# linyicheng1/keypoint_bench

Hardware: AMD Instinct MI355X
Metric: image-pairs/sec (extract+NMS+BF-match, 640x480, top_k=1000) (higher is better)
Workload: dtype f32

## Files before the change

### keypoint_bench_amd/csrc/match.hip

```cpp
#include "kpb_common.h"

namespace {

struct SampleArgs {
    const float* desc; const float* pts; const int* n; float* out;
    int C, Hd, Wd, pts_cols, max_n;
    long long sb, sc, sh, sw;
};

constexpr int SAMPLE_KPW = 4;
__global__ __launch_bounds__(256) void sample_bilinear(SampleArgs a)
{
    const int b = blockIdx.y, lane = threadIdx.x & 63;
    const int i0 = (blockIdx.x * 4 + (threadIdx.x >> 6)) * SAMPLE_KPW;
    const int n = a.n ? min(a.n[b], a.max_n) : a.max_n;
    if (i0 >= n) return;
    float cf[SAMPLE_KPW][4];
    long long off[SAMPLE_KPW][4];
    bool ok[SAMPLE_KPW][4];
#pragma unroll
    for (int k = 0; k < SAMPLE_KPW; ++k) {
        const int i = min(i0 + k, n - 1);
        const float* p = a.pts + ((size_t)b * a.max_n + i) * a.pts_cols;
        const float gx = (p[0] - 0.5f) * 2.0f, gy = (p[1] - 0.5f) * 2.0f;
        const float x = (gx + 1.0f) * ((float)(a.Wd - 1) / 2.0f), y = (gy + 1.0f) * ((float)(a.Hd - 1) / 2.0f);
        const float xw = floorf(x), yn = floorf(y);
        const float w = x - xw, e = 1.0f - w, nn = y - yn, s = 1.0f - nn;
        cf[k][0] = s * e; cf[k][1] = s * w; cf[k][2] = nn * e; cf[k][3] = nn * w;
        const long long x0 = (long long)xw, y0 = (long long)yn, x1 = x0 + 1, y1 = y0 + 1;
        const bool vx0 = x0 >= 0 && x0 < a.Wd, vx1 = x1 >= 0 && x1 < a.Wd;
        const bool vy0 = y0 >= 0 && y0 < a.Hd, vy1 = y1 >= 0 && y1 < a.Hd;
        ok[k][0] = vx0 && vy0; ok[k][1] = vx1 && vy0; ok[k][2] = vx0 && vy1; ok[k][3] = vx1 && vy1;
        off[k][0] = ok[k][0] ? y0 * a.sh + x0 * a.sw : 0; off[k][1] = ok[k][1] ? y0 * a.sh + x1 * a.sw : 0;
        off[k][2] = ok[k][2] ? y1 * a.sh + x0 * a.sw : 0; off[k][3] = ok[k][3] ? y1 * a.sh + x1 * a.sw : 0;
    }
    const float* base = a.desc + (size_t)b * a.sb;
    for (int ch = lane; ch < a.C; ch += 64) {
        const float* q = base + (size_t)ch * a.sc;
        float t[SAMPLE_KPW][4];
#pragma unroll
        for (int k = 0; k < SAMPLE_KPW; ++k)
#pragma unroll
            for (int c = 0; c < 4; ++c) t[k][c] = q[off[k][c]];
#pragma unroll
        for (int k = 0; k < SAMPLE_KPW; ++k) {
            const float nw = ok[k][0] ? t[k][0] : 0.0f, ne = ok[k][1] ? t[k][1] : 0.0f;
            const float sw = ok[k][2] ? t[k][2] : 0.0f, se = ok[k][3] ? t[k][3] : 0.0f;
            if (i0 + k < n)
                a.out[((size_t)b * a.max_n + i0 + k) * a.C + ch] =
                    __fadd_rn(__fadd_rn(__fadd_rn(__fmul_rn(nw, cf[k][0]), __fmul_rn(ne, cf[k][1])), __fmul_rn(sw, cf[k][2])), __fmul_rn(se, cf[k][3]));
        }
    }
}

__device__ __forceinline__ bool precedes(double s1, int i1, double s2, int i2)
{
    if (s1 == s2) return i1 < i2;
    const bool n1 = s1 != s1, n2 = s2 != s2;
    if (n1 | n2) return n1 && (!n2 || i1 < i2);
    const double hi = fmax(s1, s2), lo = fmin(s1, s2);
    if (hi - lo <= hi * 4.5e-16) {
        const double d1 = sqrt(s1), d2 = sqrt(s2);
        if (d1 == d2) return i1 < i2;
        return d1 < d2;
    }
    return s1 < s2;
}

constexpr int TM = 4, TN = 8;
constexpr int MTI = 16 * TM, MTJ = 16 * TN, KC = 16, MATCH_THREADS = 256;

struct MatchArgs {
    const int* only;
    const float* d0; const float* d1; const int* n; const int* m;
    double* rpart_s; int* rpart_j;
    double* cpart_s; int* cpart_i;
    int C, max_n, max_m, tiles_i, rdepth;
};

__host__ __device__ constexpr int row_depth(int tiles_j) { return 2 * tiles_j > 8 ? 2 * tiles_j : 8; }

#define COLJ(c, q) (2 * (c) + 32 * ((q) >> 1) + ((q) & 1))
template <bool RATIO>
__global__ __launch_bounds__(MATCH_THREADS) void match_tile(MatchArgs a)
{
    constexpr int PA = MTI + 2, PB = MTJ + 2;
    constexpr int STAGE = KC * (PA + PB) * 2, RED = 16 * MTJ * 3;
    __shared__ __attribute__((aligned(16))) unsigned smem[STAGE > RED ? STAGE : RED];
    double (*A)[PA] = reinterpret_cast<double (*)[PA]>(smem);
    double (*Bt)[PB] = reinterpret_cast<double (*)[PB]>(smem + KC * PA * 2);
    const int b = blockIdx.z, tj = blockIdx.x, ti = blockIdx.y, tid = threadIdx.x;
    if (a.only && !a.only[b]) return;
    const int n = a.n ? min(a.n[b], a.max_n) : a.max_n, m = a.m ? min(a.m[b], a.max_m) : a.max_m;
    const int i0 = ti * MTI, j0 = tj * MTJ;
    if (i0 >= n || j0 >= m) return;
    const float* d0 = a.d0 + (size_t)b * a.max_n * a.C;
    const float* d1 = a.d1 + (size_t)b * a.max_m * a.C;
    const int r = tid >> 4, c = tid & 15;
    double acc[TM][TN];
#pragma unroll
    for (int p = 0; p < TM; ++p)
#pragma unroll
        for (int q = 0; q < TN; ++q) acc[p][q] = 0.0;

    const bool vec = (a.C % 4) == 0;
    for (int k0 = 0; k0 < a.C; k0 += KC) {
        if (vec) {
            for (int x = tid; x < (MTI + MTJ) * (KC / 4); x += MATCH_THREADS) {
                const int row = x / (KC / 4), kq = x - row * (KC / 4), kk = k0 + 4 * kq;
                const bool second = row >= MTI;
                const int lr = second ? row - MTI : row;
                const float* src = second ? d1 + (size_t)min(j0 + lr, m - 1) * a.C : d0 + (size_t)min(i0 + lr, n - 1) * a.C;
                float4 v = make_float4(0.f, 0.f, 0.f, 0.f);
                if (kk < a.C) v = *reinterpret_cast<const float4*>(src + kk);
                double* dst = second ? &Bt[4 * kq][lr] : &A[4 * kq][lr];
                const int pitch = second ? PB : PA;
                dst[0] = (double)v.x; dst[pitch] = (double)v.y; dst[2 * pitch] = (double)v.z; dst[3 * pitch] = (double)v.w;
            }
        } else {
            for (int x = tid; x < (MTI + MTJ) * KC; x += MATCH_THREADS) {
                const int row = x % (MTI + MTJ), k = x / (MTI + MTJ), kk = k0 + k;
                if (row < MTI) A[k][row] = (kk < a.C) ? (double)d0[(size_t)min(i0 + row, n - 1) * a.C + kk] : 0.0;
                else Bt[k][row - MTI] = (kk < a.C) ? (double)d1[(size_t)min(j0 + row - MTI, m - 1) * a.C + kk] : 0.0;
            }
        }
        __syncthreads();
        const int kend = min(KC, a.C - k0);
        for (int k = 0; k < kend; ++k) {
            double av[TM], bv[TN];
#pragma unroll
            for (int p = 0; p < TM; ++p) av[p] = A[k][TM * r + p];
#pragma unroll
            for (int q = 0; q < TN; ++q) bv[q] = Bt[k][COLJ(c, q)];
#pragma unroll
            for (int p = 0; p < TM; ++p)
#pragma unroll
                for (int q = 0; q < TN; ++q) {
                    const double d = __dsub_rn(av[p], bv[q]);
                    acc[p][q] = __dadd_rn(acc[p][q], __dmul_rn(d, d));
                }
        }
        __syncthreads();
    }

    const int lane = tid & 63;
#pragma unroll
    for (int p = 0; p < TM; ++p) {
        double bs = __longlong_as_double(0x7FF0000000000000LL);
        int bj = 0x7FFFFFFF;
        double ss = bs;
        int sj = bj;
#pragma unroll
        for (int q = 0; q < TN; ++q) {
            const int j = j0 + COLJ(c, q);
            if (j < m) {
                if (precedes(acc[p][q], j, bs, bj)) {
                    if (RATIO) { ss = bs; sj = bj; }
                    bs = acc[p][q]; bj = j;
                } else if (RATIO && precedes(acc[p][q], j, ss, sj)) { ss = acc[p][q]; sj = j; }
            }
        }
#pragma unroll
        for (int d = 1; d < 16; d <<= 1) {
            const double os = __shfl_xor(bs, d, 64);
            const int oj = __shfl_xor(bj, d, 64);
            if (RATIO) {
                const double os2 = __shfl_xor(ss, d, 64);
                const int oj2 = __shfl_xor(sj, d, 64);
                if (precedes(os, oj, bs, bj)) {
                    if (precedes(os2, oj2, bs, bj)) { ss = os2; sj = oj2; } else { ss = bs; sj = bj; }
                    bs = os; bj = oj;
                } else if (precedes(os, oj, ss, sj)) { ss = os; sj = oj; }
            } else if (precedes(os, oj, bs, bj)) { bs = os; bj = oj; }
        }
        const int i = i0 + TM * r + p;
        if ((lane & 15) == 0 && i < n) {
            const size_t o = ((size_t)b * a.rdepth + (RATIO ? 2 * tj : tj)) * a.max_n + i;
            a.rpart_s[o] = bs; a.rpart_j[o] = bj;
            if (RATIO) { a.rpart_s[o + a.max_n] = ss; a.rpart_j[o + a.max_n] = sj; }
        }
    }
    double (*cs)[MTJ] = reinterpret_cast<double (*)[MTJ]>(smem);
    int (*ci)[MTJ] = reinterpret_cast<int (*)[MTJ]>(smem + 16 * MTJ * 2);
#pragma unroll
    for (int q = 0; q < TN; ++q) {
        double bs = __longlong_as_double(0x7FF0000000000000LL);
        int bi = 0x7FFFFFFF;
#pragma unroll
        for (int p = 0; p < TM; ++p) {
            const int i = i0 + TM * r + p;
            if (i < n && precedes(acc[p][q], i, bs, bi)) { bs = acc[p][q]; bi = i; }
        }
        cs[r][COLJ(c, q)] = bs; ci[r][COLJ(c, q)] = bi;
    }
    __syncthreads();
    if (tid < MTJ) {
        double bs = cs[0][tid]; int bi = ci[0][tid];
        for (int g = 1; g < 16; ++g)
            if (precedes(cs[g][tid], ci[g][tid], bs, bi)) { bs = cs[g][tid]; bi = ci[g][tid]; }
        const int j = j0 + tid;
        if (j < m) {
            const size_t o = ((size_t)b * a.tiles_i + ti) * a.max_m + j;
            a.cpart_s[o] = bs; a.cpart_i[o] = bi;
        }
    }
}

constexpr int FIN_THREADS = 1024;

struct FinArgs {
    const double* rpart_s; const int* rpart_j; const double* cpart_s; const int* cpart_i;
    const int* n; const int* m;
    int* out_pairs; double* out_dist; int* out_k;
    int* host_k;
    int max_n, max_m, tiles_i, rdepth, cross_check;
    double max_distance;
    const int* exact;
    double max_ratio;
};

template <bool RATIO>
__global__ __launch_bounds__(FIN_THREADS) void match_finalize(FinArgs a)
{
    extern __shared__ __attribute__((aligned(16))) unsigned char smem[];
    int* colarg = reinterpret_cast<int*>(smem);
    __shared__ int wsum[FIN_THREADS / 64];
    const int b = blockIdx.x, tid = threadIdx.x, lane = tid & 63, wid = tid >> 6;
    const int n = a.n ? min(a.n[b], a.max_n) : a.max_n, m = a.m ? min(a.m[b], a.max_m) : a.max_m;
    const int tiles_i = (n + MTI - 1) / MTI;
    const int rslots = !RATIO ? (m + MTJ - 1) / MTJ : (a.exact && !a.exact[b]) ? a.rdepth : 2 * ((m + MTJ - 1) / MTJ);
    for (int j = tid; j < m; j += FIN_THREADS) {
        double bs = __longlong_as_double(0x7FF0000000000000LL);
        int bi = 0x7FFFFFFF;
        for (int t = 0; t < tiles_i; ++t) {
            const size_t o = ((size_t)b * a.tiles_i + t) * a.max_m + j;
            const double s = a.cpart_s[o]; const int i = a.cpart_i[o];
            if (i != 0x7FFFFFFF && precedes(s, i, bs, bi)) { bs = s; bi = i; }
        }
        colarg[j] = bi;
    }
    __syncthreads();
    int base = 0;
    for (int c0 = 0; c0 < n; c0 += FIN_THREADS) {
        const int i = c0 + tid;
        bool keep = false;
        double dist = 0.0;
        int bj = 0;
        if (i < n && m > 0) {
            double bs = __longlong_as_double(0x7FF0000000000000LL);
            bj = 0x7FFFFFFF;
            int bt = 0;
            for (int t = 0; t < rslots; ++t) {
                const size_t o = ((size_t)b * a.rdepth + t) * a.max_n + i;
                const double s = a.rpart_s[o]; const int j = a.rpart_j[o];
                if (j != 0x7FFFFFFF && precedes(s, j, bs, bj)) { bs = s; bj = j; bt = t; }
            }
            dist = sqrt(bs);
            keep = (!a.cross_check || colarg[bj] == i) && (!(a.max_distance < __longlong_as_double(0x7FF0000000000000LL)) || dist < a.max_distance);
            if (RATIO && keep) {
                double ss = __longlong_as_double(0x7FF0000000000000LL);
                int sj = 0x7FFFFFFF;
                for (int t = 0; t < rslots; ++t) {
                    const size_t o = ((size_t)b * a.rdepth + t) * a.max_n + i;
                    const double s = a.rpart_s[o]; const int j = a.rpart_j[o];
                    if (t != bt && j != 0x7FFFFFFF && precedes(s, j, ss, sj)) { ss = s; sj = j; }
                }
                double second = sqrt(ss);
                if (second == 0.0) second = 2.220446049250313e-16;
                keep = __ddiv_rn(dist, second) < a.max_ratio;
            }
        }
        const unsigned long long bal = __ballot(keep);
        const int within = __popcll(bal & ((1ull << lane) - 1ull));
        if (lane == 0) wsum[wid] = __popcll(bal);
        __syncthreads();
        int wbase = 0, tot = 0;
        for (int w = 0; w < FIN_THREADS / 64; ++w) { const int s = wsum[w]; if (w < wid) wbase += s; tot += s; }
        __syncthreads();
        if (keep) {
            const int pos = base + wbase + within;
            a.out_pairs[((size_t)b * a.max_n + pos) * 2 + 0] = i;
            a.out_pairs[((size_t)b * a.max_n + pos) * 2 + 1] = bj;
            if (a.out_dist) a.out_dist[(size_t)b * a.max_n + pos] = dist;
        }
        base += tot;
    }
    if (tid == 0) { a.out_k[b] = base; a.host_k[b] = base; }
}

typedef _Float16 mh8 __attribute__((ext_vector_type(8)));
typedef float mf4 __attribute__((ext_vector_type(4)));
constexpr unsigned INF_BITS = 0x7F800000u;
__device__ __forceinline__ float match_margin(float na, float nb, int C)
{
    return (7.5e-6f + 6.0e-7f * (float)C) * (na + nb) + 5.0e-6f * (sqrtf(na) + sqrtf(nb));
}

struct PreArgs {
    const float* d0; const float* d1; const int* n; const int* m;
    int C, max_n, max_m;
    uint4* h0; uint4* h1;
    float* nrm0; float* nrm1;
    unsigned* rowmin; unsigned* colmin;
    int* rcnt; int* ccnt;
    int* flag;
    int* ncand;
    unsigned* nmax;
};

__global__ __launch_bounds__(256) void match_prep(PreArgs a)
{
    __shared__ unsigned s_max[2];
    const int b = blockIdx.y, tid = threadIdx.x, q = tid & 7;
    const int n = a.n ? min(a.n[b], a.max_n) : a.max_n, m = a.m ? min(a.m[b], a.max_m) : a.max_m;
    const int P8 = a.C / 8;
    if (tid < 2) s_max[tid] = 0u;
    __syncthreads();
    const int r = min(blockIdx.x * 32 + (tid >> 3), a.max_n + a.max_m - 1);
    const bool second = r >= a.max_n;
    const int row = second ? r - a.max_n : r;
    const int cnt = second ? m : n, cap = second ? a.max_m : a.max_n;
    const float* src = (second ? a.d1 : a.d0) + ((size_t)b * cap + row) * a.C;
    uint4* dst = (second ? a.h1 : a.h0) + ((size_t)b * cap + row) * P8;
    const size_t lo_off = (size_t)gridDim.y * cap * P8;
    float nn = 0.0f, big = 0.0f;
    if (row < cnt) {
        for (int p8 = q; p8 < P8; p8 += 8) {
            const float4 u = *reinterpret_cast<const float4*>(src + 8 * p8), v = *reinterpret_cast<const float4*>(src + 8 * p8 + 4);
            const float f[8] = {u.x, u.y, u.z, u.w, v.x, v.y, v.z, v.w};
            big = fmaxf(fmaxf(fmaxf(big, fmaxf(fabsf(u.x), fabsf(u.y))), fmaxf(fabsf(u.z), fabsf(u.w))),
                        fmaxf(fmaxf(fabsf(v.x), fabsf(v.y)), fmaxf(fabsf(v.z), fabsf(v.w))));
            unsigned hw[4], lw[4];
#pragma unroll
            for (int k = 0; k < 4; ++k) {
                typedef _Float16 h2 __attribute__((ext_vector_type(2)));
                const h2 hh = __builtin_bit_cast(h2, __builtin_amdgcn_cvt_pkrtz(f[2 * k], f[2 * k + 1]));
                const h2 ll = __builtin_bit_cast(h2, __builtin_amdgcn_cvt_pkrtz(f[2 * k] - (float)hh[0], f[2 * k + 1] - (float)hh[1]));
                hw[k] = __builtin_bit_cast(unsigned, hh); lw[k] = __builtin_bit_cast(unsigned, ll);
                nn = fmaf(f[2 * k], f[2 * k], nn); nn = fmaf(f[2 * k + 1], f[2 * k + 1], nn);
            }
            dst[p8] = make_uint4(hw[0], hw[1], hw[2], hw[3]);
            dst[lo_off + p8] = make_uint4(lw[0], lw[1], lw[2], lw[3]);
        }
    }
    nn += kpb_shfl_xor<1>(nn); nn += kpb_shfl_xor<2>(nn); nn += kpb_shfl_xor<4>(nn);
    if (row < cnt && big >= 32768.0f) a.flag[b] = 1;
    if (row < cnt && q == 0) {
        if (!(nn < 3.0e38f)) a.flag[b] = 1;
        else atomicMax(&s_max[second ? 1 : 0], __float_as_uint(nn));
    }
    if (q == 0) {
        (second ? a.nrm1 : a.nrm0)[(size_t)b * cap + row] = nn;
        (second ? a.colmin : a.rowmin)[(size_t)b * cap + row] = INF_BITS;
        (second ? a.ccnt : a.rcnt)[(size_t)b * cap + row] = 0;
    }
    __syncthreads();
    if (tid < 2 && s_max[tid]) atomicMax(&a.nmax[2 * b + tid], s_max[tid]);
}

struct ApxArgs {
    const uint4* h0; const uint4* h1; const float* nrm0; const float* nrm1; const int* n; const int* m;
    int max_n, max_m, P8; size_t lo0, lo1;
    unsigned* rowmin; unsigned* colmin;
    int2* cand; int* ncand; int cap; int* flag;
    const unsigned* nmax; int C;
};

constexpr int CBUF = 192;

template <int KB, int RT, int PASS, bool RATIO = false>
__global__ __launch_bounds__(256) void match_approx(ApxArgs a)
{
    static_assert(PASS == 0 || !RATIO, "the candidate pass is the same with the ratio test on");
    __shared__ int2 cbuf[PASS == 1 ? 4 : 1][PASS == 1 ? CBUF : 1];
    int wcnt = 0;
    const int b = blockIdx.y, tid = threadIdx.x, lane = tid & 63, wv = tid >> 6;
    auto flush = [&]() {
        if (PASS == 1 && wcnt > 0) {
            int base = 0;
            if (lane == 0) base = atomicAdd(&a.ncand[b], wcnt);
            base = __shfl(base, 0, 64);
            for (int i = lane; i < wcnt; i += 64) {
                if (base + i < a.cap) a.cand[(size_t)b * a.cap + base + i] = cbuf[PASS == 1 ? wv : 0][i];
                else a.flag[b] = 1;
            }
            wcnt = 0;
        }
    };
    const int n = a.n ? min(a.n[b], a.max_n) : a.max_n, m = a.m ? min(a.m[b], a.max_m) : a.max_m;
    if (a.flag[b]) return;
    const int i0 = (blockIdx.x * 4 + wv) * (16 * RT);
    if (i0 >= n) return;
    const int c16 = lane & 15, g = lane >> 4;
    const uint4* A = a.h0 + (size_t)b * a.max_n * a.P8;
    const uint4* Bm = a.h1 + (size_t)b * a.max_m * a.P8;
    mh8 ah[RT][KB], al[RT][KB];
    float na[RT][4];
#pragma unroll
    for (int rt = 0; rt < RT; ++rt) {
        const int row = min(i0 + 16 * rt + c16, n - 1);
#pragma unroll
        for (int kb = 0; kb < KB; ++kb) {
            ah[rt][kb] = __builtin_bit_cast(mh8, A[(size_t)row * a.P8 + 4 * kb + g]);
            al[rt][kb] = __builtin_bit_cast(mh8, A[a.lo0 + (size_t)row * a.P8 + 4 * kb + g]);
        }
#pragma unroll
        for (int r = 0; r < 4; ++r) {
            const int i = i0 + 16 * rt + 4 * g + r;
            na[rt][r] = i < n ? a.nrm0[(size_t)b * a.max_n + i] : __uint_as_float(INF_BITS);
        }
    }
    const float namax = __uint_as_float(a.nmax[2 * b]), nbmax = __uint_as_float(a.nmax[2 * b + 1]);
    float rmin[RT][4];
    float rmin2[RATIO ? RT : 1][4];
    if (RATIO) {
#pragma unroll
        for (int rt = 0; rt < RT; ++rt)
#pragma unroll
            for (int r = 0; r < 4; ++r) rmin2[RATIO ? rt : 0][r] = __uint_as_float(INF_BITS);
    }
#pragma unroll
    for (int rt = 0; rt < RT; ++rt)
#pragma unroll
        for (int r = 0; r < 4; ++r) rmin[rt][r] = PASS == 0 ? __uint_as_float(INF_BITS)
                                                             : (i0 + 16 * rt + 4 * g + r < n ? __uint_as_float(a.rowmin[(size_t)b * a.max_n + i0 + 16 * rt + 4 * g + r]) + match_margin(na[rt][r], nbmax, a.C) : -1.0f);
    for (int j0 = 0; j0 < m; j0 += 16) {
        const int j = j0 + c16;
        const int jr = min(j, m - 1);
        mh8 bh[KB], bl[KB];
#pragma unroll
        for (int kb = 0; kb < KB; ++kb) {
            bh[kb] = __builtin_bit_cast(mh8, Bm[(size_t)jr * a.P8 + 4 * kb + g]);
            bl[kb] = __builtin_bit_cast(mh8, Bm[a.lo1 + (size_t)jr * a.P8 + 4 * kb + g]);
        }
        const float nb = j < m ? a.nrm1[(size_t)b * a.max_m + j] : __uint_as_float(INF_BITS);
        const float cmin_j = PASS == 1 && j < m ? __uint_as_float(a.colmin[(size_t)b * a.max_m + j]) + match_margin(namax, nb, a.C) : -1.0f;
        float cm = __uint_as_float(INF_BITS);
#pragma unroll
        for (int rt = 0; rt < RT; ++rt) {
            mf4 acc = {0.f, 0.f, 0.f, 0.f};
#pragma unroll
            for (int kb = 0; kb < KB; ++kb) {
                acc = __builtin_amdgcn_mfma_f32_16x16x32_f16(al[rt][kb], bh[kb], acc, 0, 0, 0);
                acc = __builtin_amdgcn_mfma_f32_16x16x32_f16(ah[rt][kb], bl[kb], acc, 0, 0, 0);
                acc = __builtin_amdgcn_mfma_f32_16x16x32_f16(ah[rt][kb], bh[kb], acc, 0, 0, 0);
            }
            float dd[4];
#pragma unroll
            for (int r = 0; r < 4; ++r)
                dd[r] = fmaxf(__fadd_rn(__fadd_rn(na[rt][r], nb), -2.0f * acc[r]), 0.0f) + 0.0f;
            if (PASS == 0) {
#pragma unroll
                for (int r = 0; r < 4; ++r) {
                    if (RATIO) rmin2[RATIO ? rt : 0][r] = fminf(rmin2[RATIO ? rt : 0][r], fmaxf(rmin[rt][r], dd[r]));
                    rmin[rt][r] = fminf(rmin[rt][r], dd[r]); cm = fminf(cm, dd[r]);
                }
            } else {
                unsigned rowc = 0, colc = 0;
#pragma unroll
                for (int r = 0; r < 4; ++r) {
                    const bool fin = dd[r] < __uint_as_float(INF_BITS);
                    rowc |= (fin && dd[r] <= rmin[rt][r]) ? 1u << r : 0u;
                    colc |= (fin && dd[r] <= cmin_j) ? 1u << r : 0u;
                }
                const unsigned any = rowc | colc;
                if (__ballot(any != 0)) {
#pragma unroll
                    for (int r = 0; r < 4; ++r) {
                        const bool hit = (any >> r) & 1u;
                        const unsigned long long bal = __ballot(hit);
                        if (bal) {
                            if (hit) cbuf[PASS == 1 ? wv : 0][wcnt + __popcll(bal & ((1ull << lane) - 1ull))] =
                                make_int2((i0 + 16 * rt + 4 * g + r) | (((rowc >> r) & 1u) ? 1 << 30 : 0) | (((colc >> r) & 1u) ? 1 << 29 : 0), j);
                            wcnt += __popcll(bal);
                            if (wcnt > CBUF - 64) flush();
                        }
                    }
                }
            }
        }
        if (PASS == 0) {
            cm = fminf(cm, kpb_shfl_xor<16>(cm));
            cm = kpb_min32(cm);
            if (g == 0 && j < m) atomicMin(&a.colmin[(size_t)b * a.max_m + j], __float_as_uint(cm));
        }
    }
    flush();
    if (PASS == 0) {
#pragma unroll
        for (int rt = 0; rt < RT; ++rt)
#pragma unroll
            for (int r = 0; r < 4; ++r) {
                float v = rmin[rt][r];
                if (RATIO) {
                    float w = rmin2[RATIO ? rt : 0][r], ov, ow;
                    ov = kpb_shfl_xor<1>(v); ow = kpb_shfl_xor<1>(w); w = fminf(fmaxf(v, ov), fminf(w, ow)); v = fminf(v, ov);
                    ov = kpb_shfl_xor<2>(v); ow = kpb_shfl_xor<2>(w); w = fminf(fmaxf(v, ov), fminf(w, ow)); v = fminf(v, ov);
                    ov = kpb_shfl_xor<4>(v); ow = kpb_shfl_xor<4>(w); w = fminf(fmaxf(v, ov), fminf(w, ow)); v = fminf(v, ov);
                    ov = kpb_shfl_xor<8>(v); ow = kpb_shfl_xor<8>(w); w = fminf(fmaxf(v, ov), fminf(w, ow));
                    v = w;
                } else {
                    v = fminf(v, kpb_shfl_xor<1>(v)); v = fminf(v, kpb_shfl_xor<2>(v));
                    v = fminf(v, kpb_shfl_xor<4>(v)); v = fminf(v, kpb_shfl_xor<8>(v));
                }
                const int i = i0 + 16 * rt + 4 * g + r;
                if (c16 == 0 && i < n) a.rowmin[(size_t)b * a.max_n + i] = __float_as_uint(v);
            }
    }
}

struct ExactArgs {
    const float* d0; const float* d1; const int2* cand; const int* ncand; int cap, C, max_n, max_m;
    int* rcnt; int* ccnt; double* rs; int* rj; double* cs; int* ci; int tiles_i, rdepth; const int* m; const int* n; int* flag;
    int ratio;
};

__global__ __launch_bounds__(256) void match_exact(ExactArgs a)
{
    const int b = blockIdx.y;
    const int e = blockIdx.x * 256 + threadIdx.x;
    if (a.flag[b] || e >= min(a.ncand[b], a.cap)) return;
    const int2 c = a.cand[(size_t)b * a.cap + e];
    const int i = c.x & 0x1FFFFFFF, j = c.y;
    const float* pa = a.d0 + ((size_t)b * a.max_n + i) * a.C;
    const float* pb = a.d1 + ((size_t)b * a.max_m + j) * a.C;
    double s = 0.0;
    for (int k = 0; k < a.C; k += 4) {
        const float4 u = *reinterpret_cast<const float4*>(pa + k), v = *reinterpret_cast<const float4*>(pb + k);
        double d = __dsub_rn((double)u.x, (double)v.x); s = __dadd_rn(s, __dmul_rn(d, d));
        d = __dsub_rn((double)u.y, (double)v.y); s = __dadd_rn(s, __dmul_rn(d, d));
        d = __dsub_rn((double)u.z, (double)v.z); s = __dadd_rn(s, __dmul_rn(d, d));
        d = __dsub_rn((double)u.w, (double)v.w); s = __dadd_rn(s, __dmul_rn(d, d));
    }
    const int n = a.n ? min(a.n[b], a.max_n) : a.max_n, m = a.m ? min(a.m[b], a.max_m) : a.max_m;
    const int slots_r = a.ratio ? a.rdepth : (m + MTJ - 1) / MTJ, slots_c = (n + MTI - 1) / MTI;
    if (c.x & (1 << 30)) {
        const int t = atomicAdd(&a.rcnt[(size_t)b * a.max_n + i], 1);
        if (t < slots_r) { const size_t o = ((size_t)b * a.rdepth + t) * a.max_n + i; a.rs[o] = s; a.rj[o] = j; }
        else a.flag[b] = 1;
    }
    if (c.x & (1 << 29)) {
        const int t = atomicAdd(&a.ccnt[(size_t)b * a.max_m + j], 1);
        if (t < slots_c) { const size_t o = ((size_t)b * a.tiles_i + t) * a.max_m + j; a.cs[o] = s; a.ci[o] = i; }
        else a.flag[b] = 1;
    }
}

__global__ void gather_rows(const float* src, int src_rows, int cols, const int* idx, int idx_rows, int idx_stride,
                            int idx_col, const int* k, float* out)
{
    const int b = blockIdx.y;
    const int kk = k ? min(k[b], idx_rows) : idx_rows;
    const int e = blockIdx.x * blockDim.x + threadIdx.x;
    const int i = e / cols, c = e - i * cols;
    if (i >= kk) return;
    const int r = idx[((size_t)b * idx_rows + i) * idx_stride + idx_col];
    out[((size_t)b * idx_rows + i) * cols + c] = src[((size_t)b * src_rows + r) * cols + c];
}

}

extern "C" __attribute__((visibility("default"))) int kpb_sample(kpb_ctx* ctx, const float* desc_dev, int batch, int C, int Hd, int Wd, int64_t sb,
                          int64_t sc, int64_t sh, int64_t sw, const float* pts_dev, int pts_cols, int max_n,
                          const int32_t* n_dev, float* out_dev)
{
    if (!ctx) return kpb_fail(nullptr, KPB_E_INVALID, "kpb_sample: null context");
    if (max_n == 0) return KPB_OK;
    if (!desc_dev || !pts_dev || !out_dev || batch <= 0 || C <= 0 || Hd <= 0 || Wd <= 0 || pts_cols < 2 || max_n < 0)
        return kpb_fail(ctx, KPB_E_INVALID, "kpb_sample: bad argument");
    KPB_HIP(ctx, hipSetDevice(ctx->device));
    SampleArgs a{desc_dev, pts_dev, n_dev, out_dev, C, Hd, Wd, pts_cols, max_n, sb, sc, sh, sw};
    KPB_LAUNCH(ctx, "sample_bilinear", sample_bilinear, dim3(cdiv(max_n, 4 * SAMPLE_KPW), batch), dim3(256), 0, ctx->stream, a);
    KPB_HIP(ctx, hipGetLastError());
    return KPB_OK;
}

static int match_impl(kpb_ctx* ctx, const float* d0_dev, const float* d1_dev, int batch, int C, int max_n, int max_m, const int32_t* n_dev,
                      const int32_t* m_dev, const kpb_match_params* prm, double max_ratio, int32_t* out_pairs_dev, double* out_dist_dev, int32_t* out_k_dev)
{
    const bool ratio = max_ratio < 1.0;
    ctx->match_counts_valid = 0;
    if (!prm || !out_k_dev || batch <= 0 || C <= 0 || max_n < 0 || max_m < 0)
        return kpb_fail(ctx, KPB_E_INVALID, "kpb_match: bad argument");
    KPB_HIP(ctx, hipSetDevice(ctx->device));
    if (ctx->host_match_cap < batch) {
        KPB_HIP(ctx, hipStreamSynchronize(ctx->stream));
        if (ctx->host_match) KPB_HIP(ctx, hipHostFree(ctx->host_match));
        ctx->host_match = nullptr; ctx->host_match_cap = 0;
        KPB_HIP(ctx, hipHostMalloc(reinterpret_cast<void**>(&ctx->host_match), (size_t)batch * sizeof(int), hipHostMallocDefault));
        ctx->host_match_cap = batch;
    }
    ctx->host_match_n = batch;
    if (max_n == 0 || max_m == 0) {
        KPB_HIP(ctx, hipMemsetAsync(out_k_dev, 0, (size_t)batch * sizeof(int), ctx->stream));
        KPB_HIP(ctx, hipStreamSynchronize(ctx->stream));
        for (int b = 0; b < batch; ++b) ctx->host_match[b] = 0;
        ctx->match_counts_valid = 1;
        return KPB_OK;
    }
    if (!d0_dev || !d1_dev || !out_pairs_dev) return kpb_fail(ctx, KPB_E_INVALID, "kpb_match: null buffer");
    if (max_m > 16384) return kpb_fail(ctx, KPB_E_UNSUPPORTED, "kpb_match: max_m %d > 16384", max_m);
    const int tiles_i = cdiv(max_n, MTI), tiles_j = cdiv(max_m, MTJ);
    const int rdepth = ratio ? row_depth(tiles_j) : tiles_j;
    const size_t nr = (size_t)batch * rdepth * max_n, nc = (size_t)batch * tiles_i * max_m;
    double *rs = nullptr, *cs = nullptr;
    int* rj = nullptr;
    if (int rc = kpb_carve(ctx, ctx->ws_match, [&](Arena& a) { rs = a.take<double>(nr); cs = a.take<double>(nc); rj = a.take<int>(nr + nc); })) return rc;
    int* ci = rj + nr;
    static const int prefilter = kpb_env_int("KPB_MATCH_PREFILTER", 1);
    const bool pre = prefilter && (batch >= 8 || prefilter == 2) && (C % 32 == 0) && C <= 256 && tiles_i >= 2 && tiles_j >= 2 && (reinterpret_cast<uintptr_t>(d0_dev) % 16 == 0) &&
                     (reinterpret_cast<uintptr_t>(d1_dev) % 16 == 0);
    const int* only = nullptr;
    if (pre) {
        const int P8 = C / 8, cap = 8 * (max_n + max_m);
        const size_t nh0 = (size_t)batch * max_n * P8, nh1 = (size_t)batch * max_m * P8;
        const size_t n0 = (size_t)batch * max_n, n1 = (size_t)batch * max_m;
        uint4 *h0 = nullptr, *h1 = nullptr; float *nrm0 = nullptr, *nrm1 = nullptr; unsigned *rowmin = nullptr, *colmin = nullptr;
        int *rcnt = nullptr, *ccnt = nullptr, *flag = nullptr; int2* cand = nullptr;
        if (int rc = kpb_carve(ctx, ctx->ws_misc, [&](Arena& a) {
                h0 = a.take<uint4>(2 * nh0); h1 = a.take<uint4>(2 * nh1);
                nrm0 = a.take<float>(n0); nrm1 = a.take<float>(n1);
                rowmin = a.take<unsigned>(n0); colmin = a.take<unsigned>(n1);
                rcnt = a.take<int>(n0); ccnt = a.take<int>(n1);
                flag = a.take<int>(4 * (size_t)batch);
                cand = a.take<int2>((size_t)batch * cap);
            })) return rc;
        int* ncand = flag + batch;
        unsigned* nmax = reinterpret_cast<unsigned*>(ncand + batch);
        KPB_HIP(ctx, hipMemsetAsync(flag, 0, (size_t)batch * 4 * sizeof(int), ctx->stream));
        PreArgs pa{d0_dev, d1_dev, n_dev, m_dev, C, max_n, max_m, h0, h1, nrm0, nrm1, rowmin, colmin, rcnt, ccnt, flag, ncand, nmax};
        KPB_HIP(ctx, hipMemsetD32Async(reinterpret_cast<hipDeviceptr_t>(rj), 0x7FFFFFFF, nr + nc, ctx->stream));
        KPB_LAUNCH(ctx, "match_prep", match_prep, dim3(cdiv(max_n + max_m, 32), batch), dim3(256), 0, ctx->stream, pa);
        ApxArgs xa{h0, h1, nrm0, nrm1, n_dev, m_dev, max_n, max_m, P8, nh0, nh1, rowmin, colmin, cand, ncand, cap, flag, nmax, C};
        const int KB = C / 32;
#define KPB_APX(KB_, RT_)                                                                                                                   \
        {                                                                                                                                       \
            const dim3 grid(cdiv(max_n, 64 * RT_), batch);                                                                                      \
            if (ratio) KPB_LAUNCH(ctx, "match_approx_min2", (match_approx<KB_, RT_, 0, true>), grid, dim3(256), 0, ctx->stream, xa);            \
            else KPB_LAUNCH(ctx, "match_approx_min", (match_approx<KB_, RT_, 0>), grid, dim3(256), 0, ctx->stream, xa);                         \
            KPB_LAUNCH(ctx, "match_approx_cand", (match_approx<KB_, RT_, 1>), grid, dim3(256), 0, ctx->stream, xa);                             \
        }
        if (KB == 1) KPB_APX(1, 4) else if (KB == 2) KPB_APX(2, 4) else if (KB == 3) KPB_APX(3, 2) else if (KB == 4) KPB_APX(4, 2)
        else if (KB == 5) KPB_APX(5, 1) else if (KB == 6) KPB_APX(6, 1) else if (KB == 7) KPB_APX(7, 1) else KPB_APX(8, 1)
#undef KPB_APX
        ExactArgs ea{d0_dev, d1_dev, cand, ncand, cap, C, max_n, max_m, rcnt, ccnt, rs, rj, cs, ci, tiles_i, rdepth, m_dev, n_dev, flag, ratio ? 1 : 0};
        KPB_LAUNCH(ctx, "match_exact", match_exact, dim3(cdiv(cap, 256), batch), dim3(256), 0, ctx->stream, ea);
        only = flag;
    }
    MatchArgs a{only, d0_dev, d1_dev, n_dev, m_dev, rs, rj, cs, ci, C, max_n, max_m, tiles_i, rdepth};
    FinArgs f{rs, rj, cs, ci, n_dev, m_dev, out_pairs_dev, out_dist_dev, out_k_dev, ctx->host_match,
              max_n, max_m, tiles_i, rdepth, prm->cross_check, prm->max_distance, only, max_ratio};
    if (ratio) {
        KPB_LAUNCH(ctx, "match_tile2", match_tile<true>, dim3(tiles_j, tiles_i, batch), dim3(MATCH_THREADS), 0, ctx->stream, a);
        KPB_LAUNCH(ctx, "match_finalize_ratio", match_finalize<true>, dim3(batch), dim3(FIN_THREADS), (size_t)max_m * sizeof(int), ctx->stream, f);
    } else {
        KPB_LAUNCH(ctx, "match_tile", match_tile<false>, dim3(tiles_j, tiles_i, batch), dim3(MATCH_THREADS), 0, ctx->stream, a);
        KPB_LAUNCH(ctx, "match_finalize", match_finalize<false>, dim3(batch), dim3(FIN_THREADS), (size_t)max_m * sizeof(int), ctx->stream, f);
    }
    KPB_HIP(ctx, hipGetLastError());
    ctx->match_counts_valid = 1;
    return KPB_OK;
}

extern "C" __attribute__((visibility("default"))) int kpb_match(kpb_ctx* ctx, const float* d0_dev, const float* d1_dev, int batch, int C, int max_n,
                         int max_m, const int32_t* n_dev, const int32_t* m_dev, const kpb_match_params* prm,
                         int32_t* out_pairs_dev, double* out_dist_dev, int32_t* out_k_dev)
{
    if (!ctx) return kpb_fail(nullptr, KPB_E_INVALID, "kpb_match: null context");
    return match_impl(ctx, d0_dev, d1_dev, batch, C, max_n, max_m, n_dev, m_dev, prm, 1.0, out_pairs_dev, out_dist_dev, out_k_dev);
}

extern "C" __attribute__((visibility("default"))) int kpb_match_ratio(kpb_ctx* ctx, const float* d0_dev, const float* d1_dev, int batch, int C, int max_n,
                               int max_m, const int32_t* n_dev, const int32_t* m_dev, const kpb_match_params* prm, double max_ratio,
                               int32_t* out_pairs_dev, double* out_dist_dev, int32_t* out_k_dev)
{
    if (max_ratio != max_ratio) {
        if (ctx) ctx->match_counts_valid = 0;
        return kpb_fail(ctx, KPB_E_INVALID, "kpb_match_ratio: max_ratio is NaN");
    }
    if (!ctx) return kpb_fail(nullptr, KPB_E_INVALID, "kpb_match_ratio: null context");
    return match_impl(ctx, d0_dev, d1_dev, batch, C, max_n, max_m, n_dev, m_dev, prm, max_ratio, out_pairs_dev, out_dist_dev, out_k_dev);
}

extern "C" __attribute__((visibility("default"))) int kpb_match_counts(kpb_ctx* ctx, int32_t* out_k_host, int batch)
{
    if (!ctx) return kpb_fail(nullptr, KPB_E_INVALID, "kpb_match_counts: null context");
    if (!out_k_host || batch <= 0) return kpb_fail(ctx, KPB_E_INVALID, "kpb_match_counts: bad argument");
    if (!ctx->host_match || !ctx->match_counts_valid)
        return kpb_fail(ctx, KPB_E_INVALID, "kpb_match_counts: no completed match (the last kpb_match failed, was rejected, or none has run)");
    if (batch != ctx->host_match_n)
        return kpb_fail(ctx, KPB_E_INVALID, "kpb_match_counts: the last kpb_match had %d pairs, not %d", ctx->host_match_n, batch);
    KPB_HIP(ctx, hipSetDevice(ctx->device));
    KPB_HIP(ctx, kpb_wait_stream(ctx, batch < 8));
    for (int b = 0; b < batch; ++b) out_k_host[b] = ctx->host_match[b];
    return KPB_OK;
}

extern "C" __attribute__((visibility("default"))) int kpb_gather_rows(kpb_ctx* ctx, const float* src_dev, int batch, int src_rows, int cols,
                               const int32_t* idx_dev, int idx_rows, int idx_stride, int idx_col,
                               const int32_t* k_dev, float* out_dev)
{
    if (!ctx) return kpb_fail(nullptr, KPB_E_INVALID, "kpb_gather_rows: null context");
    if (idx_rows == 0) return KPB_OK;
    if (!src_dev || !idx_dev || !out_dev || batch <= 0 || cols <= 0 || idx_rows < 0 || idx_stride <= 0)
        return kpb_fail(ctx, KPB_E_INVALID, "kpb_gather_rows: bad argument");
    KPB_HIP(ctx, hipSetDevice(ctx->device));
    KPB_LAUNCH(ctx, "gather_rows", gather_rows, dim3(cdiv(idx_rows * cols, 256), batch), dim3(256), 0, ctx->stream, src_dev,
                       src_rows, cols, idx_dev, idx_rows, idx_stride, idx_col, k_dev, out_dev);
    KPB_HIP(ctx, hipGetLastError());
    return KPB_OK;
}
```

Before: 16100.

## Software-pipeline column fetches and shrink register use in approximate matcher

Restructures the approximate MFMA matching kernel. Next-column B fragments are prefetched with a double buffer and sched barriers so loads overlap compute. Per-row norms and thresholds move to shared memory for RT=4 to free VGPRs, with waves-per-EU hints added. Float min/clamp logic becomes integer min on float bits, ballots replace per-lane bitmasks, and the cross-half reduction uses permlane32_swap. The risks are extra LDS traffic, different register pressure, and subtle semantic changes in the clamping and threshold behaviour (FLT_MAX clamp, dropped max with 0).

```diff
diff --git a/keypoint_bench_amd/csrc/match.hip b/keypoint_bench_amd/csrc/match.hip
--- a/keypoint_bench_amd/csrc/match.hip
+++ b/keypoint_bench_amd/csrc/match.hip
@@ -368,9 +368,18 @@
 
 constexpr int CBUF = 192;
 
+template <int KB>
+struct ApxCol { mh8 h[KB], l[KB]; float nb; unsigned cm; };
+constexpr int FLT_MAX_BITS = 0x7F7FFFFF;
+constexpr bool apx_lookahead(int KB, int RT) { return !(KB == 2 && RT == 4); }
+constexpr int apx_waves(int KB, int RT) { return KB <= 2 && RT == 4 ? 4 : 1; }
+
 template <int KB, int RT, int PASS, bool RATIO = false>
-__global__ __launch_bounds__(256) void match_approx(ApxArgs a)
-{
+__global__ __launch_bounds__(256) __attribute__((amdgpu_waves_per_eu(apx_waves(KB, RT)))) void match_approx(ApxArgs a)
+{
+    constexpr bool LA = apx_lookahead(KB, RT);
+    constexpr bool SH = RT == 4;
+    __shared__ float4 rowd[SH ? 4 : 1][SH ? 2 : 1][SH ? RT * 4 : 1];
     static_assert(PASS == 0 || !RATIO, "the candidate pass is the same with the ratio test on");
     __shared__ int2 cbuf[PASS == 1 ? 4 : 1][PASS == 1 ? CBUF : 1];
     int wcnt = 0;
@@ -394,8 +403,37 @@
     const int c16 = lane & 15, g = lane >> 4;
     const uint4* A = a.h0 + (size_t)b * a.max_n * a.P8;
     const uint4* Bm = a.h1 + (size_t)b * a.max_m * a.P8;
+    const float namax = __uint_as_float(a.nmax[2 * b]), nbmax = __uint_as_float(a.nmax[2 * b + 1]);
+    const float inf = __uint_as_float(INF_BITS);
+    float na[SH ? 1 : RT][4];
+    float rthr[PASS == 1 && !SH ? RT : 1][4];
+    int rmin[PASS == 0 ? RT : 1][4];
+    int rmin2[RATIO && !SH ? RT : 1][4];
+    __shared__ int4 rmin2s[RATIO && SH ? RT : 1][RATIO && SH ? 256 : 1];
+#pragma unroll
+    for (int rt = 0; rt < RT; ++rt) {
+        float nv[4], tv[4];
+#pragma unroll
+        for (int r = 0; r < 4; ++r) {
+            const int i = i0 + 16 * rt + 4 * g + r;
+            nv[r] = i < n ? a.nrm0[(size_t)b * a.max_n + i] : inf;
+            tv[r] = 0.0f;
+            if (PASS == 1) {
+                const float t = i < n ? __uint_as_float(a.rowmin[(size_t)b * a.max_n + i]) + match_margin(nv[r], nbmax, a.C) : -inf;
+                tv[r] = t > __int_as_float(FLT_MAX_BITS) ? __int_as_float(FLT_MAX_BITS) : t;
+            }
+            if (PASS == 0) rmin[PASS == 0 ? rt : 0][r] = (int)INF_BITS;
+            if (RATIO && !SH) rmin2[RATIO && !SH ? rt : 0][r] = (int)INF_BITS;
+            if (!SH) { na[SH ? 0 : rt][r] = nv[r]; if (PASS == 1) rthr[PASS == 1 && !SH ? rt : 0][r] = tv[r]; }
+        }
+        if (RATIO && SH) rmin2s[RATIO && SH ? rt : 0][RATIO && SH ? tid : 0] = make_int4((int)INF_BITS, (int)INF_BITS, (int)INF_BITS, (int)INF_BITS);
+        if (SH && c16 == 0) {
+            rowd[SH ? wv : 0][0][SH ? 4 * rt + g : 0] = make_float4(nv[0], nv[1], nv[2], nv[3]);
+            if (PASS == 1) rowd[SH ? wv : 0][SH ? 1 : 0][SH ? 4 * rt + g : 0] = make_float4(tv[0], tv[1], tv[2], tv[3]);
+        }
+    }
+    if (SH) __builtin_amdgcn_wave_barrier();
     mh8 ah[RT][KB], al[RT][KB];
-    float na[RT][4];
 #pragma unroll
     for (int rt = 0; rt < RT; ++rt) {
         const int row = min(i0 + 16 * rt + c16, n - 1);
@@ -404,74 +442,83 @@
             ah[rt][kb] = __builtin_bit_cast(mh8, A[(size_t)row * a.P8 + 4 * kb + g]);
             al[rt][kb] = __builtin_bit_cast(mh8, A[a.lo0 + (size_t)row * a.P8 + 4 * kb + g]);
         }
-#pragma unroll
-        for (int r = 0; r < 4; ++r) {
-            const int i = i0 + 16 * rt + 4 * g + r;
-            na[rt][r] = i < n ? a.nrm0[(size_t)b * a.max_n + i] : __uint_as_float(INF_BITS);
-        }
-    }
-    const float namax = __uint_as_float(a.nmax[2 * b]), nbmax = __uint_as_float(a.nmax[2 * b + 1]);
-    float rmin[RT][4];
-    float rmin2[RATIO ? RT : 1][4];
-    if (RATIO) {
-#pragma unroll
-        for (int rt = 0; rt < RT; ++rt)
-#pragma unroll
-            for (int r = 0; r < 4; ++r) rmin2[RATIO ? rt : 0][r] = __uint_as_float(INF_BITS);
-    }
-#pragma unroll
-    for (int rt = 0; rt < RT; ++rt)
-#pragma unroll
-        for (int r = 0; r < 4; ++r) rmin[rt][r] = PASS == 0 ? __uint_as_float(INF_BITS)
-                                                             : (i0 + 16 * rt + 4 * g + r < n ? __uint_as_float(a.rowmin[(size_t)b * a.max_n + i0 + 16 * rt + 4 * g + r]) + match_margin(na[rt][r], nbmax, a.C) : -1.0f);
-    for (int j0 = 0; j0 < m; j0 += 16) {
+    }
+    const char* Bh = reinterpret_cast<const char*>(Bm);
+    const char* Bl = reinterpret_cast<const char*>(Bm + a.lo1);
+    const char* nbp = reinterpret_cast<const char*>(a.nrm1 + (size_t)b * a.max_m);
+    const char* cmp = reinterpret_cast<const char*>(a.colmin + (size_t)b * a.max_m);
+    auto fetch = [&](int j0, ApxCol<KB>& f) {
+        const unsigned jr = (unsigned)max(min(j0 + c16, m - 1), 0);
+        const unsigned off = (jr * (unsigned)a.P8 + (unsigned)g) * 16u;
+#pragma unroll
+        for (int kb = 0; kb < KB; ++kb) {
+            f.h[kb] = __builtin_bit_cast(mh8, *reinterpret_cast<const uint4*>(Bh + 64 * kb + off));
+            f.l[kb] = __builtin_bit_cast(mh8, *reinterpret_cast<const uint4*>(Bl + 64 * kb + off));
+        }
+        f.nb = *reinterpret_cast<const float*>(nbp + 4u * jr);
+        f.cm = PASS == 1 ? *reinterpret_cast<const unsigned*>(cmp + 4u * jr) : 0u;
+    };
+    auto step = [&](int j0, const ApxCol<KB>& f) {
         const int j = j0 + c16;
-        const int jr = min(j, m - 1);
-        mh8 bh[KB], bl[KB];
-#pragma unroll
-        for (int kb = 0; kb < KB; ++kb) {
-            bh[kb] = __builtin_bit_cast(mh8, Bm[(size_t)jr * a.P8 + 4 * kb + g]);
-            bl[kb] = __builtin_bit_cast(mh8, Bm[a.lo1 + (size_t)jr * a.P8 + 4 * kb + g]);
-        }
-        const float nb = j < m ? a.nrm1[(size_t)b * a.max_m + j] : __uint_as_float(INF_BITS);
-        const float cmin_j = PASS == 1 && j < m ? __uint_as_float(a.colmin[(size_t)b * a.max_m + j]) + match_margin(namax, nb, a.C) : -1.0f;
-        float cm = __uint_as_float(INF_BITS);
+        const float nb = j < m ? f.nb : inf;
+        float cthr = -inf;
+        if (PASS == 1) {
+            const float t = __uint_as_float(f.cm) + match_margin(namax, nb, a.C);
+            cthr = j < m ? (t > __int_as_float(FLT_MAX_BITS) ? __int_as_float(FLT_MAX_BITS) : t) : -inf;
+        }
+        int cm = (int)INF_BITS;
+        int gs = g;
+        if (SH) asm volatile("" : "+v"(gs));
+        int ts = tid;
+        if (RATIO && SH) asm volatile("" : "+v"(ts));
 #pragma unroll
         for (int rt = 0; rt < RT; ++rt) {
             mf4 acc = {0.f, 0.f, 0.f, 0.f};
 #pragma unroll
             for (int kb = 0; kb < KB; ++kb) {
-                acc = __builtin_amdgcn_mfma_f32_16x16x32_f16(al[rt][kb], bh[kb], acc, 0, 0, 0);
-                acc = __builtin_amdgcn_mfma_f32_16x16x32_f16(ah[rt][kb], bl[kb], acc, 0, 0, 0);
-                acc = __builtin_amdgcn_mfma_f32_16x16x32_f16(ah[rt][kb], bh[kb], acc, 0, 0, 0);
-            }
-            float dd[4];
-#pragma unroll
-            for (int r = 0; r < 4; ++r)
-                dd[r] = fmaxf(__fadd_rn(__fadd_rn(na[rt][r], nb), -2.0f * acc[r]), 0.0f) + 0.0f;
+                acc = __builtin_amdgcn_mfma_f32_16x16x32_f16(al[rt][kb], f.h[kb], acc, 0, 0, 0);
+                acc = __builtin_amdgcn_mfma_f32_16x16x32_f16(ah[rt][kb], f.l[kb], acc, 0, 0, 0);
+                acc = __builtin_amdgcn_mfma_f32_16x16x32_f16(ah[rt][kb], f.h[kb], acc, 0, 0, 0);
+            }
+            float x[4];
+            float nar[4], thr[4];
+            if (SH) {
+                const float4 v = rowd[SH ? wv : 0][0][SH ? 4 * rt + gs : 0];
+                nar[0] = v.x; nar[1] = v.y; nar[2] = v.z; nar[3] = v.w;
+                if (PASS == 1) { const float4 t = rowd[SH ? wv : 0][SH ? 1 : 0][SH ? 4 * rt + gs : 0]; thr[0] = t.x; thr[1] = t.y; thr[2] = t.z; thr[3] = t.w; }
+            } else {
+#pragma unroll
+                for (int r = 0; r < 4; ++r) { nar[r] = na[SH ? 0 : rt][r]; thr[r] = PASS == 1 ? rthr[PASS == 1 && !SH ? rt : 0][r] : 0.0f; }
+            }
+#pragma unroll
+            for (int r = 0; r < 4; ++r) x[r] = __builtin_fmaf(acc[r], -2.0f, __fadd_rn(nar[r], nb));
             if (PASS == 0) {
+                int w[4] = {0, 0, 0, 0};
+                if (RATIO && SH) { const int4 v = rmin2s[RATIO && SH ? rt : 0][RATIO && SH ? ts : 0]; w[0] = v.x; w[1] = v.y; w[2] = v.z; w[3] = v.w; }
 #pragma unroll
                 for (int r = 0; r < 4; ++r) {
-                    if (RATIO) rmin2[RATIO ? rt : 0][r] = fminf(rmin2[RATIO ? rt : 0][r], fmaxf(rmin[rt][r], dd[r]));
-                    rmin[rt][r] = fminf(rmin[rt][r], dd[r]); cm = fminf(cm, dd[r]);
+                    const int xi = __float_as_int(x[r]);
+                    if (RATIO && !SH) w[r] = rmin2[RATIO && !SH ? rt : 0][r];
+                    if (RATIO) w[r] = min(w[r], max(rmin[PASS == 0 ? rt : 0][r], xi));
+                    if (RATIO && !SH) rmin2[RATIO && !SH ? rt : 0][r] = w[r];
+                    rmin[PASS == 0 ? rt : 0][r] = min(rmin[PASS == 0 ? rt : 0][r], xi); cm = min(cm, xi);
                 }
+                if (RATIO && SH) rmin2s[RATIO && SH ? rt : 0][RATIO && SH ? ts : 0] = make_int4(w[0], w[1], w[2], w[3]);
+                if (SH && (rt & 1)) __builtin_amdgcn_sched_barrier(0);
             } else {
-                unsigned rowc = 0, colc = 0;
+                unsigned long long rowm[4], colm[4], any = 0ull;
 #pragma unroll
                 for (int r = 0; r < 4; ++r) {
-                    const bool fin = dd[r] < __uint_as_float(INF_BITS);
-                    rowc |= (fin && dd[r] <= rmin[rt][r]) ? 1u << r : 0u;
-                    colc |= (fin && dd[r] <= cmin_j) ? 1u << r : 0u;
+                    rowm[r] = __ballot(x[r] <= thr[r]); colm[r] = __ballot(x[r] <= cthr);
+                    any |= rowm[r] | colm[r];
                 }
-                const unsigned any = rowc | colc;
-                if (__ballot(any != 0)) {
+                if (any) {
 #pragma unroll
                     for (int r = 0; r < 4; ++r) {
-                        const bool hit = (any >> r) & 1u;
-                        const unsigned long long bal = __ballot(hit);
+                        const unsigned long long bal = rowm[r] | colm[r];
                         if (bal) {
-                            if (hit) cbuf[PASS == 1 ? wv : 0][wcnt + __popcll(bal & ((1ull << lane) - 1ull))] =
-                                make_int2((i0 + 16 * rt + 4 * g + r) | (((rowc >> r) & 1u) ? 1 << 30 : 0) | (((colc >> r) & 1u) ? 1 << 29 : 0), j);
+                            if ((bal >> lane) & 1ull) cbuf[PASS == 1 ? wv : 0][wcnt + __popcll(bal & ((1ull << lane) - 1ull))] =
+                                make_int2((i0 + 16 * rt + 4 * gs + r) | (((rowm[r] >> lane) & 1ull) ? 1 << 30 : 0) | (((colm[r] >> lane) & 1ull) ? 1 << 29 : 0), j);
                             wcnt += __popcll(bal);
                             if (wcnt > CBUF - 64) flush();
                         }
@@ -480,9 +527,31 @@
             }
         }
         if (PASS == 0) {
-            cm = fminf(cm, kpb_shfl_xor<16>(cm));
-            cm = kpb_min32(cm);
-            if (g == 0 && j < m) atomicMin(&a.colmin[(size_t)b * a.max_m + j], __float_as_uint(cm));
+            cm = min(cm, kpb_shfl_xor<16>(cm));
+            const auto hv = __builtin_amdgcn_permlane32_swap((unsigned)cm, (unsigned)cm, false, false);
+            cm = max(min((int)hv[0], (int)hv[1]), 0);
+            if (g == 0 && j < m) atomicMin(&a.colmin[(size_t)b * a.max_m + j], (unsigned)cm);
+        }
+    };
+    if (LA) {
+        ApxCol<KB> f0, f1;
+        fetch(0, f0);
+        for (int j0 = 0; j0 < m; j0 += 32) {
+            fetch(j0 + 16, f1);
+            __builtin_amdgcn_sched_barrier(0);
+            step(j0, f0);
+            __builtin_amdgcn_sched_barrier(0);
+            if (j0 + 16 >= m) break;
+            fetch(j0 + 32, f0);
+            __builtin_amdgcn_sched_barrier(0);
+            step(j0 + 16, f1);
+            __builtin_amdgcn_sched_barrier(0);
+        }
+    } else {
+        for (int j0 = 0; j0 < m; j0 += 16) {
+            ApxCol<KB> f;
+            fetch(j0, f);
+            step(j0, f);
         }
     }
     flush();
@@ -491,20 +560,20 @@
         for (int rt = 0; rt < RT; ++rt)
 #pragma unroll
             for (int r = 0; r < 4; ++r) {
-                float v = rmin[rt][r];
+                int v = rmin[PASS == 0 ? rt : 0][r];
                 if (RATIO) {
-                    float w = rmin2[RATIO ? rt : 0][r], ov, ow;
-                    ov = kpb_shfl_xor<1>(v); ow = kpb_shfl_xor<1>(w); w = fminf(fmaxf(v, ov), fminf(w, ow)); v = fminf(v, ov);
-                    ov = kpb_shfl_xor<2>(v); ow = kpb_shfl_xor<2>(w); w = fminf(fmaxf(v, ov), fminf(w, ow)); v = fminf(v, ov);
-                    ov = kpb_shfl_xor<4>(v); ow = kpb_shfl_xor<4>(w); w = fminf(fmaxf(v, ov), fminf(w, ow)); v = fminf(v, ov);
-                    ov = kpb_shfl_xor<8>(v); ow = kpb_shfl_xor<8>(w); w = fminf(fmaxf(v, ov), fminf(w, ow));
+                    int w = SH ? (&rmin2s[RATIO && SH ? rt : 0][RATIO && SH ? tid : 0].x)[r] : rmin2[RATIO && !SH ? rt : 0][r], ov, ow;
+                    ov = kpb_shfl_xor<1>(v); ow = kpb_shfl_xor<1>(w); w = min(max(v, ov), min(w, ow)); v = min(v, ov);
+                    ov = kpb_shfl_xor<2>(v); ow = kpb_shfl_xor<2>(w); w = min(max(v, ov), min(w, ow)); v = min(v, ov);
+                    ov = kpb_shfl_xor<4>(v); ow = kpb_shfl_xor<4>(w); w = min(max(v, ov), min(w, ow)); v = min(v, ov);
+                    ov = kpb_shfl_xor<8>(v); ow = kpb_shfl_xor<8>(w); w = min(max(v, ov), min(w, ow));
                     v = w;
                 } else {
-                    v = fminf(v, kpb_shfl_xor<1>(v)); v = fminf(v, kpb_shfl_xor<2>(v));
-                    v = fminf(v, kpb_shfl_xor<4>(v)); v = fminf(v, kpb_shfl_xor<8>(v));
+                    v = min(v, kpb_shfl_xor<1>(v)); v = min(v, kpb_shfl_xor<2>(v));
+                    v = min(v, kpb_shfl_xor<4>(v)); v = min(v, kpb_shfl_xor<8>(v));
                 }
                 const int i = i0 + 16 * rt + 4 * g + r;
-                if (c16 == 0 && i < n) a.rowmin[(size_t)b * a.max_n + i] = __float_as_uint(v);
+                if (c16 == 0 && i < n) a.rowmin[(size_t)b * a.max_n + i] = (unsigned)max(v, 0);
             }
     }
 }
```

Result: no change. 16050 (-0.3%).
